# dfm/emcee

Hardware: AMD Instinct MI355X
Metric: walker-updates/sec (whole node), 64-dim correlated Gaussian, StretchMove a=2 (higher is better)
Workload: dtype f64

## Files before the change

### emcee_amd/csrc/emx_kernels.hpp

```cpp
#pragma once
#include <hip/hip_runtime.h>

#include <cstdint>
#include <type_traits>

#include "emx_planlog.hpp"
#include "emx_rng.hpp"

#ifndef EMX_OPT_RED4
#define EMX_OPT_RED4 1
#endif
#ifndef EMX_OPT_RTILE
#define EMX_OPT_RTILE 1
#endif
#ifndef EMX_LEAN_FOLD_D
#define EMX_LEAN_FOLD_D 0
#endif
#ifndef EMX_LEAN_FOLD_SPW
#define EMX_LEAN_FOLD_SPW 1
#endif
#ifndef EMX_OPT_SKEW
#define EMX_OPT_SKEW 1
#endif
#ifndef EMX_SNOOKER_BUDGET
// ... 684 lines not shown
                dst_[e_] = reinterpret_cast<const double2*>(A.tp1)[e_];      \
            __syncthreads();                                                                        \
            stage_pending = false;                                                                  \
        }                                                                                           \
    } while (0)
    const int t_hi = thidev_ ? *thidev_ : A.t_hi;
    if (tlo_ + wave * spw >= t_hi) {
        EMX_STAGE_PUBLISH();
        return;
    }
    for (int t0 = tlo_ + wave * spw; t0 < t_hi; t0 += nwaves * spw) {
        const int nslot = min(spw, t_hi - t0);
        const int npass = (nslot + WPW - 1) / WPW;
        const int pbase = A.pos0 + t0;

        for (int pb = 0; pb < npass; pb += PF) {
            if (skew && stager && stage_pending) {
                EMX_STAGE_PUBLISH();
                for (int r_ = 0; r_ < skewsl_; ++r_) __builtin_amdgcn_s_sleep(8);
            }
            int wi[PF], ja[PF], jb[NR >= 3 ? PF : 1], jc[NR >= 4 ? PF : 1];
#pragma unroll
            for (int k = 0; k < PF; ++k) {
                const int srow = (pb + k) * WPW + sub;
                const int pos = pbase + (srow < nslot ? srow : 0);
                wi[k] = A.order[pos];
                if constexpr (NR >= 2) ja[k] = A.p0[pos];
                if constexpr (NR >= 3) jb[k] = A.p1[pos];
                if constexpr (NR >= 4) jc[k] = A.p2[pos];
            }
            EMX_STAMP(1);
            if (EMX_OPT_STAMPS && A.dbg) {
                asm volatile("s_waitcnt vmcnt(0)" ::: "memory");
                EMX_STAMP(13);
            }
            Row<G, V, CH> xi[PF], xa[NR >= 2 ? PF : 1], xb[NR >= 3 ? PF : 1], xc[NR >= 4 ? PF : 1];
            Row<G, V, CH> qk[RTILE ? PF : 1];
            double s0v[PF], facv[PF], lpov[PF], loguv[PF];
#pragma unroll
            for (int k = 0; k < PF; ++k) {
                const int srow = (pb + k) * WPW + sub;
                const int pos = pbase + (srow < nslot ? srow : 0);
                if (!(ablate_ & 32)) load_row<G, V, CH>(xi[k], A.X + (size_t)wi[k] * D, D, gl);
                if constexpr (MOVE == MOVE_GAUSS) {
                    if (disp_) load_row<G, V, CH>(xa[k], disp_ + (size_t)wi[k] * D, D, gl);
                } else if constexpr (NR >= 2) {
                    if (!(ablate_ & 32)) load_row<G, V, CH>(xa[k], partner_base<LEAN>(A, ja[k]) + (size_t)ja[k] * D, D, gl);
                }
                if constexpr (NR >= 3) load_row<G, V, CH>(xb[k], partner_base<LEAN>(A, jb[k]) + (size_t)jb[k] * D, D, gl);
                if constexpr (NR >= 4) load_row<G, V, CH>(xc[k], partner_base<LEAN>(A, jc[k]) + (size_t)jc[k] * D, D, gl);
                if constexpr (MOVE != MOVE_EVAL) {
                    s0v[k] = (MOVE == MOVE_SNOOKER) ? 0.0 : A.s0[pos];
                    facv[k] = A.fac[pos];
                    if (!DENSE || target_ == TGT_NONE) {
                        lpov[k] = A.lp[wi[k]];
                        loguv[k] = A.logu[pos];
                    } else {
                        lpov[k] = 0.0;
                        loguv[k] = 0.0;
                    }
                } else {
                    s0v[k] = facv[k] = lpov[k] = loguv[k] = 0.0;
                }
            }

            EMX_STAMP(2);
            if (stage_pending) EMX_STAGE_PUBLISH();
            EMX_STAMP(3);

            if (ablate_ & 128) {
                double sink = 0.0;
#pragma unroll
                for (int k = 0; k < PF; ++k) sink += xi[k].x[0][0] + xa[NR >= 2 ? k : 0].x[0][0] + lpov[k];
                if (sink == 1.2345e-300) A.fout[0] = sink;
                continue;
            }
#pragma unroll
            for (int k = 0; k < PF; ++k) {
                const int p = pb + k;
                if (p < npass) {
                    const int srow = p * WPW + sub;
                    const bool live = srow < nslot;
                    const int i = wi[k];
                    double factor = facv[k];

                    Row<G, V, CH> q;
                    if constexpr (MOVE == MOVE_GAUSS)
                        if (!disp_) gauss_disp_row<G, V, CH>(xa[k], A, i, ja[k], D, gl);
                    make_proposal<G, V, CH, MOVE>(xi[k], xa[NR >= 2 ? k : 0], xb[NR >= 3 ? k : 0], xc[NR >= 4 ? k : 0],
                                                  s0v[k], A.gammas, D, gl, q, factor, NR >= 2 ? ja[k] : -1);

                    bool badq = false;
                    if constexpr (MOVE != MOVE_EVAL) {
                        bool bl = false;
#pragma unroll
                        for (int c = 0; c < CH; ++c)
#pragma unroll
                            for (int v = 0; v < V; ++v) bl |= !(fabs(q.x[c][v]) <= 1.79769313486231570815e308);
                        badq = group_any<G>(bl, sub);
                        if (live && badq && gl == 0) raise_status(A.status, ST_BAD_COORD);
                    }

                    if (target_ == TGT_NONE) {
                        if (live) {
                            const int t = t0 + srow;
                            store_row<G, V, CH>(q, A.qout + (size_t)t * D, D, gl);
                            if (gl == 0) A.fout[t] = factor;
                        }
                    } else if (LEAN != 1 && !DENSE && target_ == TGT_REPLAY) {
                        if constexpr (MOVE != MOVE_EVAL) {
                            if (live) {
                                store_row<G, V, CH>(q, A.X + (size_t)i * D, D, gl);
                                if (gl == 0) A.lp[i] = loguv[k];
                            }
                        }
                    } else if constexpr (!DENSE) {
                        const double lp_new = eval_valu_target<G, V, CH>(q, mu, iv, A.tp0, A.tp1, target_, A.tscale, D, gl, lane);
                        if (live && gl == 0 && (lp_new != lp_new)) raise_status(A.status, ST_NAN_LOGP);
                        if constexpr (MOVE == MOVE_EVAL) {
                            if (live && gl == 0) A.lp[i] = lp_new;
                        } else {
                            const double lp_old = lpov[k];
                            const double lnpdiff = factor + lp_new - lp_old;
                            const bool accept = live && !badq && (lnpdiff > loguv[k]);
                            if (accept) {
                                store_row<G, V, CH>(q, A.X + (size_t)i * D, D, gl);
                                if (gl == 0) A.lp[i] = lp_new;
                            }
                            if (live && gl == 0) {
                                A.acc[i] = accept ? 1 : 0;
                                if (chain_lp_) {
                                    chain_lp_[i] = accept ? lp_new : lp_old;
                                    if (accept) A.acc_count[i] += 1u;
                                }
                                if (declp_) put_decision(t0 + srow - tlo_, accept ? lp_new : __builtin_nan(""));
                            }
                            if (live && chain_) store_row_stream<G, V, CH>(accept ? q : xi[k], chain_ + (size_t)i * D, D, gl);
                            if (live && sendbuf_) {
                                double* sb = sendbuf_ + (size_t)(t0 + srow - tlo_) * (D + 2);
                                store_row<G, V, CH>(accept ? q : xi[k], sb, D, gl);
                                if (gl == 0) {
                                    sb[D] = accept ? lp_new : lp_old;
                                    sb[D + 1] = accept ? 1.0 : 0.0;
                                }
                            }
                        }
                    } else {
                        const int trow = srow & 15;
#pragma unroll
                        for (int c = 0; c < CH; ++c)
#pragma unroll
                            for (int v = 0; v < V; ++v) {
                                const int d = (c * G + gl) * V + v;
                                if constexpr (RTILE) {
                                    if (d < Dp && !(ablate_ & 4)) tile[trow * RT + d] = (live && !badq) ? q.x[c][v] - mu.x[c][v] : 0.0;
                                } else {
                                    if (d < Dp && !(ablate_ & 4)) tile[trow * RT + d] = (live && !badq) ? q.x[c][v] : muS[d];
                                }
                            }
                        if constexpr (RTILE) qk[k] = q;
                        if (gl == 0) facS[trow] = badq ? -__builtin_inf() : factor;
                        if constexpr (MOVE != MOVE_EVAL) {
                            if (live && chain_) store_row_stream<G, V, CH>(xi[k], chain_ + (size_t)i * D, D, gl);
                            if (live && sendbuf_)
                                store_row<G, V, CH>(xi[k], sendbuf_ + (size_t)(t0 + srow - tlo_) * (D + 2), D, gl);
                        }
                    }
                }
            }

            EMX_STAMP(4);
            if constexpr (DENSE) {
                const int plast = (pb + PF < npass ? pb + PF : npass) - 1;
                const bool tile_done = ((plast + 1) % PPT == 0) || (plast + 1 == npass);
                if (target_ != TGT_NONE && tile_done && !(ablate_ & 16)) {
                    const int tb = (plast / PPT) * 16;
                    const int myrow = (lane >> 4) + 4 * (lane & 3);
                    const bool mine = (lane & 15) < 4 && tb + myrow < nslot;
                    const int mypos = pbase + (tb + myrow < nslot ? tb + myrow : 0);
                    const int my_i = A.order[mypos];
                    double my_lpo = 0.0, my_logu = 0.0;
                    if constexpr (MOVE != MOVE_EVAL) {
                        my_lpo = A.lp[my_i];
                        my_logu = A.logu[mypos];
                    }
                    EMX_WAVE_SYNC();
                    double my_qf = 0.0;
                    {
                        const int am = lane & 15, ak = lane >> 4;
                        typedef double d4 __attribute__((ext_vector_type(4)));
                        double afr[KK];
#pragma unroll
                        for (int kk = 0; kk < KK; ++kk) {
                            if constexpr (RTILE)
                                afr[kk] = tile[am * RT + 4 * kk + ak];
                            else
                                afr[kk] = tile[am * RT + 4 * kk + ak] - muS[4 * kk + ak];
                        }
                        double part[4] = {0.0, 0.0, 0.0, 0.0};
                        if (EMX_OPT_STAMPS && A.dbg) { asm volatile("s_waitcnt lgkmcnt(0)" ::: "memory"); }
                        EMX_STAMP(5);
                        if (!(ablate_ & 1))
#pragma unroll
                        for (int nb = 0; nb < DPB; ++nb) {
                            d4 accv = {0.0, 0.0, 0.0, 0.0};
#pragma unroll
                            for (int kk = 4 * nb; kk < KK; ++kk)
                                accv = __builtin_amdgcn_mfma_f64_16x16x4f64(afr[kk], Sfrag[(dense_block(DPB, nb, kk >> 2) * 4 + (kk & 3)) * 64 + lane], accv, 0, 0, 0);
#pragma unroll
                            for (int r = 0; r < 4; ++r) part[r] = fma(accv[r], accv[r], part[r]);
                        }
                        if (EMX_OPT_STAMPS && A.dbg) { asm volatile("s_nop 0" ::: "memory"); }
                        EMX_STAMP(6);
#if EMX_OPT_RED4
                        my_qf = row16_sum4(part[0], part[1], part[2], part[3], lane);
#else
#pragma unroll
                        for (int r = 0; r < 4; ++r) part[r] = group_sum<16>(part[r]);
                        my_qf = part[0];
#pragma unroll
                        for (int r = 1; r < 4; ++r) my_qf = (am == r) ? part[r] : my_qf;
#endif
                    }
                    EMX_STAMP(7);
                    bool acc = false;
                    double lp_fin = my_lpo;
                    if (mine) {
                        const double lpn = -0.5 * my_qf;
                        if (lpn != lpn) raise_status(A.status, ST_NAN_LOGP);
                        if constexpr (MOVE == MOVE_EVAL) {
                            A.lp[my_i] = lpn;
                        } else {
                            const double lnpdiff = facS[myrow] + lpn - my_lpo;
                            acc = lnpdiff > my_logu;
                            A.acc[my_i] = acc ? 1 : 0;
                            if (acc) {
                                A.lp[my_i] = lpn;
                                lp_fin = lpn;
                            }
                            if (chain_lp_) {
                                chain_lp_[my_i] = lp_fin;
                                if (acc) A.acc_count[my_i] += 1u;
                            }
                            if (declp_) put_decision(t0 + tb + myrow - tlo_, acc ? lpn : __builtin_nan(""));
                        }
                    }
                    EMX_STAMP(8);
                    if constexpr (MOVE != MOVE_EVAL) {
                        const unsigned long long am64 = __ballot(acc);
                        if (sendbuf_ && (lane & 15) < 4) qfS[myrow] = lp_fin;
                        if (sendbuf_) EMX_WAVE_SYNC();
#pragma unroll
                        for (int pp = 0; pp < PPT; ++pp) {
                            if (ablate_ & 8) break;
                            const int row = pp * WPW + sub;
                            const int sidx = tb + row;
                            const bool lv = sidx < nslot;
                            const bool ac = lv && ((am64 >> ((row & 3) * 16 + (row >> 2))) & 1ull);
                            if (!lv) continue;
                            if (sendbuf_ && gl == 0) {
                                double* sb = sendbuf_ + (size_t)(t0 + sidx - tlo_) * (D + 2);
                                sb[D] = qfS[row];
                                sb[D + 1] = ac ? 1.0 : 0.0;
                            }
                            if (!ac) continue;
                            int wi2;
                            if constexpr (PF == PPT) {
                                wi2 = wi[0];
#pragma unroll
                                for (int k2 = 1; k2 < PF; ++k2) wi2 = (pp == k2) ? wi[k2] : wi2;
                            } else {
                                wi2 = A.order[pbase + sidx];
                            }
                            Row<G, V, CH> rr;
                            if constexpr (RTILE) {
                                rr = qk[pp < PF ? pp : 0];
                            } else {
#pragma unroll
                                for (int c = 0; c < CH; ++c)
#pragma unroll
                                    for (int v = 0; v < V; ++v) {
                                        const int d = (c * G + gl) * V + v;
                                        rr.x[c][v] = d < D ? tile[row * RT + d] : 0.0;
                                    }
                            }
                            store_row<G, V, CH>(rr, A.X + (size_t)wi2 * D, D, gl);
                            if (chain_) store_row_stream<G, V, CH>(rr, chain_ + (size_t)wi2 * D, D, gl);
                            if (sendbuf_) store_row<G, V, CH>(rr, sendbuf_ + (size_t)(t0 + sidx - tlo_) * (D + 2), D, gl);
                        }
                    }
                    EMX_STAMP(9);
                    EMX_WAVE_SYNC();
                }
            }
        }
    }
    if (EMX_OPT_STAMPS && A.dbg) { asm volatile("s_waitcnt vmcnt(0)" ::: "memory"); }
    EMX_STAMP(10);
    if (EMX_OPT_STAMPS && A.dbg && wib == 0 && lane == 0) A.dbg[(size_t)blockIdx.x * 16 + 12] = wall_clock64();
}

typedef unsigned int emx_u4 __attribute__((ext_vector_type(4)));
constexpr int EMX_CPOL_SC1 = 16;
template <int G, int V, int CH, int CPOL = EMX_CPOL_SC1>
__device__ __forceinline__ void load_row_agent(Row<G, V, CH>& r, __amdgpu_buffer_rsrc_t rsrc, int row, int D, int gl) {
    static_assert(V == 2 || V == 1, "two coordinates per lane and chunk (even ndim), or one (odd ndim: rows are 8-byte aligned only)");
    const int base = row * D;
    if constexpr (V == 1) {
        typedef unsigned int emx_u2 __attribute__((ext_vector_type(2)));
#pragma unroll
        for (int c = 0; c < CH; ++c) {
            const int d = c * G + gl;
            if (d < D) {
                const emx_u2 w = __builtin_amdgcn_raw_buffer_load_b64(rsrc, (base + d) * 8, 0, CPOL);
                double t;
                __builtin_memcpy(&t, &w, 8);
                r.x[c][0] = t;
            } else {
                r.x[c][0] = 0.0;
            }
        }
        return;
    }
#pragma unroll
    for (int c = 0; c < CH; ++c) {
        const int d = (c * G + gl) * V;
        if (d + 1 < D) {
            const emx_u4 w = __builtin_amdgcn_raw_buffer_load_b128(rsrc, (base + d) * 8, 0, CPOL);
            double2 t;
            __builtin_memcpy(&t, &w, 16);
            r.x[c][0] = t.x;
            r.x[c][1] = t.y;
        } else {
            r.x[c][0] = 0.0;
            r.x[c][1] = 0.0;
        }
    }
}
template <int G, int V, int CH, int CPOL = EMX_CPOL_SC1>
__device__ __forceinline__ void store_row_agent(const Row<G, V, CH>& r, __amdgpu_buffer_rsrc_t rsrc, int row, int D, int gl) {
    static_assert(V == 2 || V == 1, "two coordinates per lane and chunk (even ndim), or one (odd ndim)");
    const int base = row * D;
    if constexpr (V == 1) {
        typedef unsigned int emx_u2 __attribute__((ext_vector_type(2)));
#pragma unroll
        for (int c = 0; c < CH; ++c) {
            const int d = c * G + gl;
            if (d < D) {
                emx_u2 w;
                const double t = r.x[c][0];
                __builtin_memcpy(&w, &t, 8);
                __builtin_amdgcn_raw_buffer_store_b64(w, rsrc, (base + d) * 8, 0, CPOL);
            }
        }
        return;
    }
#pragma unroll
    for (int c = 0; c < CH; ++c) {
        const int d = (c * G + gl) * V;
        if (d + 1 < D) {
            const double2 t = {r.x[c][0], r.x[c][1]};
            emx_u4 w;
            __builtin_memcpy(&w, &t, 16);
            __builtin_amdgcn_raw_buffer_store_b128(w, rsrc, (base + d) * 8, 0, CPOL);
        }
    }
}
template <typename T>
__device__ __forceinline__ void store_agent(T* p, T v) { __hip_atomic_store(p, v, __ATOMIC_RELAXED, __HIP_MEMORY_SCOPE_AGENT); }
__device__ __forceinline__ double load_agent(const double* p) { return __hip_atomic_load(p, __ATOMIC_RELAXED, __HIP_MEMORY_SCOPE_AGENT); }
__device__ __forceinline__ unsigned load_agent(const unsigned* p) { return __hip_atomic_load(p, __ATOMIC_RELAXED, __HIP_MEMORY_SCOPE_AGENT); }
template <bool LOCAL, typename T>
__device__ __forceinline__ void store_scope(T* p, T v) {
    if constexpr (LOCAL)
        *p = v;
    else
        store_agent(p, v);
}

constexpr int PERSIST_MAX_ITERS = 40;
constexpr int PERSIST_BAR_STRIDE = 32;
constexpr int PERSIST_BAR_WORDS = 12 * PERSIST_BAR_STRIDE;
struct PersistIter {
    const char* plan;
    double *chain, *chain_lp;
    int32_t pos0, split;
    double gammas;
    int32_t kind, shift;
};
struct PersistCols {
    const int32_t *order, *p0, *p1, *p2;
    const double *s0, *logu, *fac;
    double *chain, *chain_lp;
    int32_t pos0, split;
    double gammas;
    int32_t kind, shift;
    __host__ __device__ __forceinline__ PersistCols(const PersistIter& it, size_t N)
        : order(reinterpret_cast<const int32_t*>(it.plan)), p0(reinterpret_cast<const int32_t*>(it.plan) + N),
          p1(reinterpret_cast<const int32_t*>(it.plan + N * 24)), p2(reinterpret_cast<const int32_t*>(it.plan + N * 24) + N),
          s0(reinterpret_cast<const double*>(it.plan + N * 8)), logu(reinterpret_cast<const double*>(it.plan + N * 32)),
          fac(reinterpret_cast<const double*>(it.plan + N * 32) + N), chain(it.chain), chain_lp(it.chain_lp), pos0(it.pos0), split(it.split),
          gammas(it.gammas), kind(it.kind), shift(it.shift) {}
};
struct PersistArgs {
    HalfStepArgs base;
    PersistIter it[PERSIST_MAX_ITERS];
    unsigned* bar;
    unsigned* ver;
    unsigned epoch0;
    unsigned lepoch0;
    unsigned hepoch0;
    unsigned long long timeout_ticks;
    int32_t niter;
    unsigned seq;
    unsigned* started_host;
    int32_t stagger;
};
static_assert(sizeof(PersistArgs) <= 4096, "kernel arguments of the persistent kernels");

__device__ __forceinline__ void persist_barrier_local(const PersistArgs& P, unsigned k, unsigned bid, unsigned ngroups) {
    asm volatile("s_waitcnt vmcnt(0)" ::: "memory");
    __syncthreads();
    if (threadIdx.x < 64) {
        const int lane = threadIdx.x;
        const __amdgpu_buffer_rsrc_t Fr = __builtin_amdgcn_make_buffer_rsrc((void*)(P.bar + 10 * PERSIST_BAR_STRIDE), 0, 64 * 4, 0x00020000);
        if (lane == 0) __builtin_amdgcn_raw_buffer_store_b32(k, Fr, (int)bid * 4, 0, 0);
        const unsigned long long t0 = wall_clock64();
        for (;;) {
            const unsigned v = __builtin_amdgcn_raw_buffer_load_b32(Fr, lane * 4, 0, EMX_CPOL_SC1);
            const bool ok = lane < (int)ngroups ? (int)(v - k) >= 0 : true;
            const bool dead = lane == 32 && v != 0u;
            if (__ballot(ok) == ~0ull || __ballot(dead) != 0ull) break;
            if (wall_clock64() - t0 > P.timeout_ticks) {
                if (lane == 0) {
                    raise_status(P.base.status, ST_EXCHANGE_TIMEOUT);
                    __hip_atomic_store(P.bar + 9 * PERSIST_BAR_STRIDE + 1, 2u, __ATOMIC_RELAXED, __HIP_MEMORY_SCOPE_AGENT);
                    __builtin_amdgcn_raw_buffer_store_b32(1u, Fr, 32 * 4, 0, 0);
                }
                break;
            }
        }
    }
    __syncthreads();
}

__device__ __forceinline__ void persist_barrier(const PersistArgs& P, unsigned k, unsigned long long* wall = nullptr) {
    asm volatile("s_waitcnt vmcnt(0)" ::: "memory");
    __syncthreads();
    if (threadIdx.x == 0) {
        const int xcd = blockIdx.x & 7;
        const unsigned per = (gridDim.x + 7 - xcd) / 8;
        unsigned* xctr = P.bar + xcd * PERSIST_BAR_STRIDE;
        unsigned* gctr = P.bar + 8 * PERSIST_BAR_STRIDE;
        unsigned* go = P.bar + 9 * PERSIST_BAR_STRIDE;
        if (wall) wall[0] = wall_clock64();
        const unsigned old = __hip_atomic_fetch_add(xctr, 1u, __ATOMIC_RELAXED, __HIP_MEMORY_SCOPE_AGENT);
        if (old == k * per - 1) {
            const unsigned o2 = __hip_atomic_fetch_add(gctr, 1u, __ATOMIC_RELAXED, __HIP_MEMORY_SCOPE_AGENT);
            if (o2 == k * 8 - 1) __hip_atomic_store(go, k, __ATOMIC_RELAXED, __HIP_MEMORY_SCOPE_AGENT);
        }
        const unsigned long long t0 = wall_clock64();
        for (;;) {
            const unsigned long long v = __hip_atomic_load(reinterpret_cast<unsigned long long*>(go), __ATOMIC_RELAXED, __HIP_MEMORY_SCOPE_AGENT);
            if ((int)((unsigned)v - k) >= 0 || (v >> 32) != 0ull) break;
            if (wall_clock64() - t0 > P.timeout_ticks) {
                raise_status(P.base.status, ST_EXCHANGE_TIMEOUT);
                __hip_atomic_store(go + 1, 2u, __ATOMIC_RELAXED, __HIP_MEMORY_SCOPE_AGENT);
                break;
            }
        }
        if (wall) wall[1] = wall_clock64();
    }
    __syncthreads();
}

__device__ __forceinline__ void persist_stagger_wait(int stagger, int wib) {
    const int how = stagger >> 8, cnt = stagger & 255;
    const int units = how == 0 ? (wib >> 2) : how == 1 ? (wib & 1) : how == 2 ? ((wib >> 1) & 1) : (wib & 3);
    for (int s = 0; s < cnt * units; ++s) __builtin_amdgcn_s_sleep(1);
}

template <bool LOCAL = false>
__device__ __forceinline__ bool persist_handshake(const PersistArgs& P) {
    __shared__ int ok_s;
    if (threadIdx.x == 0) {
        const unsigned k = LOCAL ? P.hepoch0 + 1u : P.epoch0 + 1u;
        const int xcd = LOCAL ? 0 : (int)(blockIdx.x & 7);
        const unsigned per = LOCAL ? gridDim.x >> 3 : (gridDim.x + 7 - xcd) / 8;
        unsigned* xctr = P.bar + xcd * PERSIST_BAR_STRIDE;
        unsigned* gctr = P.bar + 8 * PERSIST_BAR_STRIDE;
        unsigned* go = P.bar + 9 * PERSIST_BAR_STRIDE;
        int ok = 1;
        const unsigned long long v0 = __hip_atomic_load(reinterpret_cast<unsigned long long*>(go), __ATOMIC_RELAXED, __HIP_MEMORY_SCOPE_AGENT);
        if ((v0 >> 32) != 0ull) {
            ok = 0;
        } else {
            unsigned xcc = 0;
            if constexpr (LOCAL) {
                asm volatile("s_getreg_b32 %0, hwreg(HW_REG_XCC_ID)" : "=s"(xcc));
                __hip_atomic_fetch_or(go + 2, 1u << (xcc & 15u), __ATOMIC_RELAXED, __HIP_MEMORY_SCOPE_AGENT);
                asm volatile("s_waitcnt vmcnt(0)" ::: "memory");
            }
            const unsigned old = __hip_atomic_fetch_add(xctr, 1u, __ATOMIC_RELAXED, __HIP_MEMORY_SCOPE_AGENT);
            if (old == k * per - 1) {
                bool open = true;
                unsigned o2 = k * 8 - 1;
                if constexpr (LOCAL) {
                    const unsigned m = __hip_atomic_load(go + 2, __ATOMIC_RELAXED, __HIP_MEMORY_SCOPE_AGENT);
                    open = (m & (m - 1u)) == 0u;
                    if (open) {
                        __hip_atomic_store(go + 2, 0u, __ATOMIC_RELAXED, __HIP_MEMORY_SCOPE_AGENT);
                    } else {
                        raise_status(P.base.status, ST_EXCHANGE_TIMEOUT);
                        __hip_atomic_store(go + 1, 1u, __ATOMIC_RELAXED, __HIP_MEMORY_SCOPE_AGENT);
                    }
                } else {
                    o2 = __hip_atomic_fetch_add(gctr, 1u, __ATOMIC_RELAXED, __HIP_MEMORY_SCOPE_AGENT);
                }
                if (open && o2 == k * 8 - 1) {
                    __hip_atomic_store(go + 4, LOCAL ? (xcc & 15u) + 1u : 0u, __ATOMIC_RELAXED, __HIP_MEMORY_SCOPE_AGENT);
                    __hip_atomic_store(go + 3, P.seq, __ATOMIC_RELAXED, __HIP_MEMORY_SCOPE_AGENT);
                    if (P.started_host) __hip_atomic_store(P.started_host, P.seq, __ATOMIC_RELAXED, __HIP_MEMORY_SCOPE_SYSTEM);
                    __hip_atomic_store(go, k, __ATOMIC_RELAXED, __HIP_MEMORY_SCOPE_AGENT);
                }
            }
            const unsigned long long t0 = wall_clock64();
            for (;;) {
                const unsigned long long v = __hip_atomic_load(reinterpret_cast<unsigned long long*>(go), __ATOMIC_RELAXED, __HIP_MEMORY_SCOPE_AGENT);
                if ((v >> 32) != 0ull) {
                    ok = 0;
                    break;
                }
                if ((int)((unsigned)v - k) >= 0) break;
                if (wall_clock64() - t0 > P.timeout_ticks) {
                    raise_status(P.base.status, ST_EXCHANGE_TIMEOUT);
                    __hip_atomic_store(go + 1, 1u, __ATOMIC_RELAXED, __HIP_MEMORY_SCOPE_AGENT);
                    ok = 0;
                    break;
                }
            }
        }
        ok_s = ok;
    }
    __syncthreads();
    return ok_s != 0;
}

template <int G, int V, int CH, int DPB, int MOVE = MOVE_STRETCH, bool LOCAL = false, bool ROWS_LATE = false>
static __global__ __launch_bounds__(512) void k_persist(const PersistArgs P) {
    static_assert(MOVE == MOVE_STRETCH || MOVE == MOVE_DE || MOVE == MOVE_SNOOKER, "the red / blue moves");
    if (LOCAL && (blockIdx.x & 7u) != 0u) return;
    const unsigned bid = LOCAL ? blockIdx.x >> 3 : blockIdx.x, ngroups = LOCAL ? gridDim.x >> 3 : gridDim.x;
    constexpr int CPOL = EMX_CPOL_SC1;
    constexpr int CPOL_ST = LOCAL ? 0 : EMX_CPOL_SC1;
    constexpr bool DE = MOVE == MOVE_DE || MOVE == MOVE_SNOOKER;
    constexpr bool SN = MOVE == MOVE_SNOOKER;
    constexpr bool DEFER = !DE;
    constexpr int WPW = 64 / G;
    constexpr int PPT = 16 / WPW;
    constexpr int PF = PPT;
    static_assert(EMX_OPT_RTILE && EMX_OPT_RED4, "the persistent kernel is the one-tile-per-batch form");
    constexpr int Dp = DPB * 16, KK = Dp / 4, RT = Dp + 2;
    static_assert(G * V * CH >= Dp, "row layout must cover the padded dimension");
    extern __shared__ __attribute__((aligned(16))) double smem[];
    const HalfStepArgs& A = P.base;
    const int lane = threadIdx.x & 63;
    const int wib = threadIdx.x >> 6;
    const int sub = lane / G;
    const int gl = lane % G;
    const int D = A.D;
    double* Sfrag = smem;
    double* muS = smem + dense_img_doubles(Dp);
    double* tile = muS + Dp + (size_t)wib * (16 * RT + 32);
    double* qfS = tile + 16 * RT;
    double* facS = qfS + 16;
    {
        constexpr int IMG2 = (dense_img_doubles(Dp) + Dp) / 2;
        const double2* img = reinterpret_cast<const double2*>(A.tp1);
        double2* dst = reinterpret_cast<double2*>(smem);
        for (int e = threadIdx.x; e < IMG2; e += blockDim.x) dst[e] = img[e];
    }
    Row<G, V, CH> mu;
    load_row<G, V, CH>(mu, A.tp0, D, gl);
    if (!persist_handshake<LOCAL>(P)) return;
    const int wave = (int)bid * (blockDim.x >> 6) + wib;
    const int t0 = wave * 16;
    unsigned long long pst[6] = {0, 0, 0, 0, 0, 0}, pt = 0;
    const bool prof = EMX_OPT_STAMPS && A.dbg && wib == EMX_STAMP_WAVE;
    if (prof) {
        pt = __builtin_readcyclecounter();
        if (lane == 0) A.dbg[(size_t)bid * 16 + 11] = wall_clock64();
    }
#define EMX_PSTAMP(k_)                                                   \
    do {                                                                 \
        if (prof) {                                                      \
            const unsigned long long t_ = __builtin_readcyclecounter(); \
            pst[k_] += t_ - pt;                                          \
            pt = t_;                                                     \
        }                                                                \
    } while (0)
    const __amdgpu_buffer_rsrc_t Xr = __builtin_amdgcn_make_buffer_rsrc((void*)A.X, 0, A.N * D * 8, 0x00020000);
    const int myrow = (lane >> 4) + 4 * (lane & 3);
    const bool mine = (lane & 15) < 4;

    int wi[PF], ja[PF], jb[DE ? PF : 1], jc[SN ? PF : 1], my_i;
    double s0v[PF], facv[PF], my_logu, my_lpo;
    Row<G, V, CH> xi[PF];
    {
        const PersistCols I(P.it[0], (size_t)P.base.N);
        const int pbase = I.pos0 + t0;
#pragma unroll
        for (int k = 0; k < PF; ++k) {
            const int pos = pbase + k * WPW + sub;
            wi[k] = I.order[pos];
            ja[k] = I.p0[pos];
            if constexpr (DE) jb[k] = I.p1[pos];
            if constexpr (SN) jc[k] = I.p2[pos];
            s0v[k] = SN ? 0.0 : I.s0[pos];
            facv[k] = I.fac[pos];
        }
        my_i = I.order[pbase + myrow];
        my_logu = I.logu[pbase + myrow];
#pragma unroll
        for (int k = 0; k < PF; ++k) load_row_agent<G, V, CH, CPOL>(xi[k], Xr, wi[k], D, gl);
        my_lpo = load_agent(A.lp + my_i);
    }
    Row<G, V, CH> crow[DEFER ? PF : 1];
    int cwi[PF], cmy_i = 0;
    double clp = 0.0;
    double *cchain = nullptr, *cchain_lp = nullptr;
#pragma unroll
    for (int k = 0; k < PF; ++k) {
        if (DEFER || k == 0) crow[DEFER ? k : 0] = xi[k];
        cwi[k] = 0;
    }
    for (int n = 0; n < P.niter; ++n) {
        const PersistCols I(P.it[n], (size_t)P.base.N);
        Row<G, V, CH> xa[PF], xb[DE ? PF : 1], xc[SN ? PF : 1];
        persist_stagger_wait(P.stagger, wib);
#pragma unroll
        for (int k = 0; k < PF; ++k) {
            load_row_agent<G, V, CH, CPOL>(xa[k], Xr, ja[k], D, gl);
            if constexpr (DE) load_row_agent<G, V, CH, CPOL>(xb[k], Xr, jb[k], D, gl);
            if constexpr (SN) load_row_agent<G, V, CH, CPOL>(xc[k], Xr, jc[k], D, gl);
        }
        const bool more = n + 1 < P.niter;
        const PersistCols J(P.it[more ? n + 1 : n], (size_t)P.base.N);
        const bool pre = more && J.split != 0;
        const unsigned stamp = P.epoch0 + (unsigned)n + 1u;
        int wi_n[PF], ja_n[PF], jb_n[DE ? PF : 1], jc_n[SN ? PF : 1], my_i_n;
        double s0_n[PF], fac_n[PF], my_logu_n;
        {
            const int pbase = J.pos0 + t0;
#pragma unroll
            for (int k = 0; k < PF; ++k) {
                const int pos = pbase + k * WPW + sub;
                wi_n[k] = J.order[pos];
                ja_n[k] = J.p0[pos];
                if constexpr (DE) jb_n[k] = J.p1[pos];
                if constexpr (SN) jc_n[k] = J.p2[pos];
                s0_n[k] = SN ? 0.0 : J.s0[pos];
                fac_n[k] = J.fac[pos];
            }
            my_i_n = J.order[pbase + myrow];
            my_logu_n = J.logu[pbase + myrow];
        }
        if (prof) { asm volatile("s_waitcnt vmcnt(0)" ::: "memory"); }
        EMX_PSTAMP(0);
        Row<G, V, CH> qk[PF];
#pragma unroll
        for (int k = 0; k < PF; ++k) {
            const int srow = k * WPW + sub;
            double factor = facv[k];
            Row<G, V, CH> q;
            make_proposal<G, V, CH, MOVE>(xi[k], xa[k], xb[DE ? k : 0], xc[SN ? k : 0], s0v[k], A.gammas, D, gl, q, factor, ja[k]);
            bool bl = false;
#pragma unroll
            for (int c = 0; c < CH; ++c)
#pragma unroll
                for (int v = 0; v < V; ++v) bl |= !(fabs(q.x[c][v]) <= 1.79769313486231570815e308);
            const bool badq = group_any<G>(bl, sub);
            if (badq && gl == 0) raise_status(A.status, ST_BAD_COORD);
            const int trow = srow & 15;
#pragma unroll
            for (int c = 0; c < CH; ++c)
#pragma unroll
                for (int v = 0; v < V; ++v) {
                    const int d = (c * G + gl) * V + v;
                    if (d < Dp) tile[trow * RT + d] = !badq ? q.x[c][v] - mu.x[c][v] : 0.0;
                }
            qk[k] = q;
            if (gl == 0) facS[trow] = badq ? -__builtin_inf() : factor;
        }
        if (DEFER && cchain) {
#pragma unroll
            for (int k = 0; k < PF; ++k) store_row_stream<G, V, CH>(crow[k], cchain + (size_t)cwi[k] * D, D, gl);
            if (mine) cchain_lp[cmy_i] = clp;
            cchain = nullptr;
        }
        if (I.chain) {
#pragma unroll
            for (int k = 0; k < PF; ++k) {
                if constexpr (DEFER)
                    crow[k] = xi[k];
                else
                    store_row_stream<G, V, CH>(xi[k], I.chain + (size_t)wi[k] * D, D, gl);
            }
        }
        double my_lpo_n = 0.0;
        if (!ROWS_LATE && more) {
#pragma unroll
            for (int k = 0; k < PF; ++k) load_row_agent<G, V, CH, CPOL>(xi[k], Xr, wi_n[k], D, gl);
            my_lpo_n = load_agent(A.lp + my_i_n);
        }
        EMX_WAVE_SYNC();
        EMX_PSTAMP(1);
        double my_qf;
        {
            const int am = lane & 15, ak = lane >> 4;
            typedef double d4 __attribute__((ext_vector_type(4)));
            double afr[KK];
#pragma unroll
            for (int kk = 0; kk < KK; ++kk) afr[kk] = tile[am * RT + 4 * kk + ak];
            double part[4] = {0.0, 0.0, 0.0, 0.0};
#pragma unroll
            for (int nb = 0; nb < DPB; ++nb) {
                d4 accv = {0.0, 0.0, 0.0, 0.0};
#pragma unroll
                for (int kk = 4 * nb; kk < KK; ++kk)
                    accv = __builtin_amdgcn_mfma_f64_16x16x4f64(afr[kk], Sfrag[(dense_block(DPB, nb, kk >> 2) * 4 + (kk & 3)) * 64 + lane], accv, 0, 0, 0);
#pragma unroll
                for (int r = 0; r < 4; ++r) part[r] = fma(accv[r], accv[r], part[r]);
            }
            my_qf = row16_sum4(part[0], part[1], part[2], part[3], lane);
        }
        if (ROWS_LATE && more) {
            __builtin_amdgcn_sched_barrier(0);
#pragma unroll
            for (int k = 0; k < PF; ++k) load_row_agent<G, V, CH, CPOL>(xi[k], Xr, wi_n[k], D, gl);
            my_lpo_n = load_agent(A.lp + my_i_n);
            __builtin_amdgcn_sched_barrier(0);
        }
        if (prof) { asm volatile("s_nop 0" ::: "memory"); }
        EMX_PSTAMP(2);
        bool acc = false;
        if (mine) {
            const double lpn = -0.5 * my_qf;
            if (lpn != lpn) raise_status(A.status, ST_NAN_LOGP);
            const double lnpdiff = facS[myrow] + lpn - my_lpo;
            acc = lnpdiff > my_logu;
            store_scope<LOCAL>(A.acc + my_i, (uint8_t)(acc ? 1 : 0));
            if (acc) {
                store_scope<LOCAL>(A.lp + my_i, lpn);
                store_scope<LOCAL>(P.ver + my_i, stamp);
            }
            if (I.chain_lp) {
                if constexpr (DEFER)
                    clp = acc ? lpn : my_lpo;
                else
                    I.chain_lp[my_i] = acc ? lpn : my_lpo;
                if (acc) store_scope<LOCAL>(A.acc_count + my_i, load_agent(A.acc_count + my_i) + 1u);
            }
        }
        const unsigned long long am64 = __ballot(acc);
#pragma unroll
        for (int pp = 0; pp < PPT; ++pp) {
            const int row = pp * WPW + sub;
            const bool ac = (am64 >> ((row & 3) * 16 + (row >> 2))) & 1ull;
            if (ac) {
                store_row_agent<G, V, CH, CPOL_ST>(qk[pp], Xr, wi[pp], D, gl);
                if (I.chain) {
                    if constexpr (DEFER)
                        crow[pp] = qk[pp];
                    else
                        store_row_stream<G, V, CH>(qk[pp], I.chain + (size_t)wi[pp] * D, D, gl);
                }
            }
        }
        if (DEFER && I.chain) {
            cchain = I.chain;
            cchain_lp = I.chain_lp;
            cmy_i = my_i;
#pragma unroll
            for (int k = 0; k < PF; ++k) cwi[k] = wi[k];
        }
        EMX_WAVE_SYNC();
        EMX_PSTAMP(3);
        if (prof) {
            asm volatile("s_waitcnt vmcnt(0)" ::: "memory");
            EMX_PSTAMP(4);
        }
        if (!more) break;
        if constexpr (LOCAL)
            persist_barrier_local(P, P.lepoch0 + (unsigned)n + 1u, bid, ngroups);
        else
            persist_barrier(P, P.epoch0 + (unsigned)n + 2u,
                            (EMX_OPT_STAMPS && A.dbg) ? A.dbg + 4096 + ((size_t)n * ngroups + bid) * 2 : nullptr);
        EMX_PSTAMP(5);
#pragma unroll
        for (int k = 0; k < PF; ++k) {
            wi[k] = wi_n[k];
            ja[k] = ja_n[k];
            if constexpr (DE) jb[k] = jb_n[k];
            if constexpr (SN) jc[k] = jc_n[k];
            s0v[k] = s0_n[k];
            facv[k] = fac_n[k];
        }
        my_i = my_i_n;
        my_logu = my_logu_n;
        my_lpo = my_lpo_n;
        if (!pre) {
            unsigned vk[PF];
#pragma unroll
            for (int k = 0; k < PF; ++k) vk[k] = load_agent(P.ver + wi[k]);
            const unsigned vm = load_agent(P.ver + my_i);
#pragma unroll
            for (int k = 0; k < PF; ++k)
                if (vk[k] == stamp) load_row_agent<G, V, CH, CPOL>(xi[k], Xr, wi[k], D, gl);
            if (vm == stamp) my_lpo = load_agent(A.lp + my_i);
        }
    }
    if (DEFER && cchain) {
#pragma unroll
        for (int k = 0; k < PF; ++k) store_row_stream<G, V, CH>(crow[k], cchain + (size_t)cwi[k] * D, D, gl);
        if (mine) cchain_lp[cmy_i] = clp;
    }
    if (prof && lane == 0) {
        unsigned long long* o = A.dbg + (size_t)bid * 16;
#pragma unroll
        for (int k = 0; k < 6; ++k) o[k] = pst[k];
        o[6] = (unsigned long long)P.niter;
        o[12] = wall_clock64();
    }
#undef EMX_PSTAMP
}

constexpr int SMALL_MAX_MOVES = 8;
struct GaussGen {
    unsigned long long gseed, gstep;
    double gfac, gsigma;
    const double* gscale;
};
constexpr int PERSIST_GAUSS_MAX_STEPS = 16;
struct PersistGaussStep {
    const int32_t* p0;
    const double* logu;
    double *chain, *chain_lp;
    unsigned long long gstep;
    double gfac;
};
struct PersistGaussArgs {
    HalfStepArgs base;
    PersistGaussStep st[PERSIST_GAUSS_MAX_STEPS];
    int32_t nsteps;
};

template <int G, int V, int CH, int DPB>
static __global__ __launch_bounds__(512) void k_persist_gauss(const PersistGaussArgs P) {
    constexpr int MOVE = MOVE_GAUSS;
    constexpr int WPW = 64 / G;
    constexpr int PPT = 16 / WPW;
    constexpr int Dp = DPB * 16, KK = Dp / 4, RT = Dp + 2;
    static_assert(EMX_OPT_RTILE && EMX_OPT_RED4 && G * V * CH >= Dp, "the one-tile-per-batch form");
    extern __shared__ __attribute__((aligned(16))) double smem[];
    const HalfStepArgs& A = P.base;
    const int lane = threadIdx.x & 63;
    const int wib = threadIdx.x >> 6;
    const int sub = lane / G;
    const int gl = lane % G;
    const int D = A.D;
    double* Sfrag = smem;
    double* muS = smem + dense_img_doubles(Dp);
    double* tile = muS + Dp + (size_t)wib * (16 * RT + 32);
    double* facS = tile + 16 * RT + 16;
    {
        constexpr int IMG2 = (dense_img_doubles(Dp) + Dp) / 2;
        const double2* img = reinterpret_cast<const double2*>(A.tp1);
        double2* dst = reinterpret_cast<double2*>(smem);
        for (int e = threadIdx.x; e < IMG2; e += blockDim.x) dst[e] = img[e];
    }
    Row<G, V, CH> mu;
    load_row<G, V, CH>(mu, A.tp0, D, gl);
    __syncthreads();
    const int wave = blockIdx.x * (blockDim.x >> 6) + wib;
    const int w0 = wave * 16;
    const int myrow = (lane >> 4) + 4 * (lane & 3);
    const bool mine = (lane & 15) < 4;
    const int my_i = w0 + myrow;
    Row<G, V, CH> xi[PPT];
#pragma unroll
    for (int k = 0; k < PPT; ++k) load_row<G, V, CH>(xi[k], A.X + (size_t)(w0 + k * WPW + sub) * D, D, gl);
    double my_lp = A.lp[my_i];
    bool my_acc = false;
    for (int s = 0; s < P.nsteps; ++s) {
        const PersistGaussStep& S = P.st[s];
        GaussGen gg;
        gg.gseed = A.gseed;
        gg.gstep = S.gstep;
        gg.gfac = S.gfac;
        gg.gsigma = A.gsigma;
        gg.gscale = A.gscale;
        const double my_logu = S.logu[my_i];
        Row<G, V, CH> qk[PPT];
#pragma unroll
        for (int k = 0; k < PPT; ++k) {
            const int i = w0 + k * WPW + sub;
            const int col = S.p0[i];
            Row<G, V, CH> xa, q;
            gauss_disp_row<G, V, CH>(xa, gg, i, col, D, gl);
            double factor = 0.0;
            make_proposal<G, V, CH, MOVE>(xi[k], xa, xa, xa, 0.0, A.gammas, D, gl, q, factor, col);
            bool bl = false;
#pragma unroll
            for (int c = 0; c < CH; ++c)
#pragma unroll
                for (int v = 0; v < V; ++v) bl |= !(fabs(q.x[c][v]) <= 1.79769313486231570815e308);
            const bool badq = group_any<G>(bl, sub);
            if (badq && gl == 0) raise_status(A.status, ST_BAD_COORD);
            const int trow = (k * WPW + sub) & 15;
#pragma unroll
            for (int c = 0; c < CH; ++c)
#pragma unroll
                for (int v = 0; v < V; ++v) {
                    const int d = (c * G + gl) * V + v;
                    if (d < Dp) tile[trow * RT + d] = !badq ? q.x[c][v] - mu.x[c][v] : 0.0;
                }
            qk[k] = q;
            if (gl == 0) facS[trow] = badq ? -__builtin_inf() : factor;
        }
        EMX_WAVE_SYNC();
        double my_qf;
        {
            const int am = lane & 15, ak = lane >> 4;
            typedef double d4 __attribute__((ext_vector_type(4)));
            double afr[KK];
#pragma unroll
            for (int kk = 0; kk < KK; ++kk) afr[kk] = tile[am * RT + 4 * kk + ak];
            double part[4] = {0.0, 0.0, 0.0, 0.0};
#pragma unroll
            for (int nb = 0; nb < DPB; ++nb) {
                d4 accv = {0.0, 0.0, 0.0, 0.0};
#pragma unroll
                for (int kk = 4 * nb; kk < KK; ++kk)
                    accv = __builtin_amdgcn_mfma_f64_16x16x4f64(afr[kk], Sfrag[(dense_block(DPB, nb, kk >> 2) * 4 + (kk & 3)) * 64 + lane], accv, 0, 0, 0);
#pragma unroll
                for (int r = 0; r < 4; ++r) part[r] = fma(accv[r], accv[r], part[r]);
            }
            my_qf = row16_sum4(part[0], part[1], part[2], part[3], lane);
        }
        bool acc = false;
        if (mine) {
            const double lpn = -0.5 * my_qf;
            if (lpn != lpn) raise_status(A.status, ST_NAN_LOGP);
            const double lnpdiff = facS[myrow] + lpn - my_lp;
            acc = lnpdiff > my_logu;
            if (acc) my_lp = lpn;
            my_acc = acc;
            if (S.chain_lp) {
                S.chain_lp[my_i] = my_lp;
                if (acc) A.acc_count[my_i] += 1u;
            }
        }
        const unsigned long long am64 = __ballot(acc);
#pragma unroll
        for (int pp = 0; pp < PPT; ++pp) {
            const int row = pp * WPW + sub;
            const bool ac = (am64 >> ((row & 3) * 16 + (row >> 2))) & 1ull;
            if (ac) xi[pp] = qk[pp];
            if (S.chain) store_row_stream<G, V, CH>(xi[pp], S.chain + (size_t)(w0 + row) * D, D, gl);
        }
        EMX_WAVE_SYNC();
    }
#pragma unroll
    for (int k = 0; k < PPT; ++k) store_row<G, V, CH>(xi[k], A.X + (size_t)(w0 + k * WPW + sub) * D, D, gl);
    if (mine) {
        A.lp[my_i] = my_lp;
        A.acc[my_i] = my_acc ? 1 : 0;
    }
}

constexpr int SMALL_ANY_MOVE = 7;

__host__ __device__ inline int native_move_choice(uint64_t seed, uint64_t step, const double* cdf, int n) {
    const Philox4 r = philox4x32_10((uint32_t)step, (uint32_t)(step >> 32), 0x4d4f5645u , 0, (uint32_t)seed,
                                    (uint32_t)(seed >> 32));
    const double u = u53(r.v[0], r.v[1]);
    int k = 0;
    while (k < n - 1 && u >= cdf[k]) ++k;
    return k;
}

struct SmallRunArgs {
    double* X;
    double* lp;
    uint8_t* acc;
    uint32_t* acc_count;
    uint32_t* status;
    double* chain;
    double* chain_lp;
    const double* tp0;
    const double* tp1;
    double tscale;
    double a[SMALL_MAX_MOVES], sigma[SMALL_MAX_MOVES], g0[SMALL_MAX_MOVES], gammas[SMALL_MAX_MOVES], cdf[SMALL_MAX_MOVES];
    int32_t kind[SMALL_MAX_MOVES], nsplits[SMALL_MAX_MOVES];
    int32_t gmode[SMALL_MAX_MOVES];
    double gsigma[SMALL_MAX_MOVES];
    const double* gscale[SMALL_MAX_MOVES];
    const double* step_fac;
    const int32_t* step_col;
    int32_t nmoves;
    unsigned long long seed, step0;
    long long i0;
    int32_t N, D, target, nsteps, thin_by, store;
    int32_t batch;
    const char* plans;
    const int32_t* step_moves;
    const unsigned long long* seeds;
    const double* tscales;
    long long tp0_stride, tp1_stride, cap;
    int32_t eval0;
    const void* user;
    int32_t stage_rows;
};

constexpr int SMALL_STATUS_WORDS = 8;

template <bool BATCH>
struct SmallMember {
    const SmallRunArgs& A;
    __device__ __forceinline__ size_t m() const { return BATCH ? (size_t)blockIdx.x : 0; }
    __device__ __forceinline__ double* X() const { return A.X + m() * (size_t)A.N * A.D; }
    __device__ __forceinline__ double* lp() const { return A.lp + m() * (size_t)A.N; }
    __device__ __forceinline__ uint8_t* acc() const { return A.acc + m() * (size_t)A.N; }
    __device__ __forceinline__ uint32_t* acc_count() const { return A.acc_count + m() * (size_t)A.N; }
    __device__ __forceinline__ uint32_t* status() const { return A.status + m() * SMALL_STATUS_WORDS; }
    __device__ __forceinline__ double* chain() const { return A.chain + m() * (size_t)A.cap * A.N * A.D; }
    __device__ __forceinline__ double* chain_lp() const { return A.chain_lp + m() * (size_t)A.cap * A.N; }
    __device__ __forceinline__ const double* tp0() const { return BATCH && A.tp0 ? A.tp0 + m() * (size_t)A.tp0_stride : A.tp0; }
    __device__ __forceinline__ const double* tp1() const { return BATCH && A.tp1 ? A.tp1 + m() * (size_t)A.tp1_stride : A.tp1; }
    __device__ __forceinline__ const double* step_fac() const { return BATCH && A.step_fac ? A.step_fac + m() * (size_t)A.nsteps : A.step_fac; }
    __device__ __forceinline__ double tscale() const { return BATCH ? A.tscales[m()] : A.tscale; }
    __device__ __forceinline__ unsigned long long seed() const { return BATCH ? A.seeds[m()] : A.seed; }
};

template <int MOVE>
__device__ __forceinline__ void small_plan_entry(const NativeArgs& na, int N, int D, int S, int pos, double a, double sigma,
                                                 double g0, int& i, int& a0, int& a1, int& a2, double& z, double& lu, double& fc) {
    int split = 0, t = pos;
    const SplitSizes sz = split_sizes(N, S);
    for (int k = 0; k < S; ++k) {
        const int n = sz.of(k);
        if (t < n) { split = k; break; }
        t -= n;
    }
    double u;
    native_slot<MOVE>(na, N, S, split, t, a, sigma, g0, i, a0, a1, a2, z, u);
    lu = plan_log_uniform(u);
    fc = (MOVE == MOVE_STRETCH) ? ((double)D - 1.0) * plan_log(z) : 0.0;
}

template <int G, int V, int CH, int MOVE, typename Member>
__device__ __forceinline__ void small_propose(const Member& M, const double* Xs, bool live, int i, int j0, int j1, int j2,
                                              double s0, double fac, double gammas, int D, int gl, int sub, Row<G, V, CH>& q,
                                              double& factor, bool& badq, const GaussGen* gg = nullptr) {
    constexpr int NR = rows_per_pass<MOVE>();
    Row<G, V, CH> xi, xa, xb, xc;
    load_row<G, V, CH>(xi, Xs + (size_t)i * D, D, gl);
    if constexpr (MOVE == MOVE_GAUSS)
        gauss_disp_row<G, V, CH>(xa, *gg, i, j0, D, gl);
    else
        load_row<G, V, CH>(xa, Xs + (size_t)j0 * D, D, gl);
    if constexpr (NR >= 3) load_row<G, V, CH>(xb, Xs + (size_t)j1 * D, D, gl);
    if constexpr (NR >= 4) load_row<G, V, CH>(xc, Xs + (size_t)j2 * D, D, gl);
    factor = fac;
    make_proposal<G, V, CH, MOVE>(xi, xa, NR >= 3 ? xb : xa, NR >= 4 ? xc : xa, (MOVE == MOVE_SNOOKER) ? 0.0 : s0, gammas, D,
                                  gl, q, factor, MOVE == MOVE_GAUSS ? j0 : -1);
    bool bl = false;
#pragma unroll
    for (int c = 0; c < CH; ++c)
#pragma unroll
        for (int v = 0; v < V; ++v) bl |= !(fabs(q.x[c][v]) <= 1.79769313486231570815e308);
    badq = group_any<G>(bl, sub);
    if (live && badq && gl == 0) raise_status(M.status(), ST_BAD_COORD);
}

template <int G, int V, int CH, int MOVE, typename Member>
__device__ __forceinline__ void small_update(const SmallRunArgs& A, const Member& M, double* Xs, double* lps, uint8_t* accs, bool live, int i,
                                             int j0, int j1, int j2, double s0, double fac, double logu, double gammas,
                                             const Row<G, V, CH>& mu, const Row<G, V, CH>& iv, int D, int gl, int sub, int lane,
                                             const GaussGen* gg = nullptr) {
    Row<G, V, CH> q;
    double factor;
    bool badq;
    small_propose<G, V, CH, MOVE>(M, Xs, live, i, j0, j1, j2, s0, fac, gammas, D, gl, sub, q, factor, badq, gg);
    const double lp_new = eval_valu_target<G, V, CH>(q, mu, iv, M.tp0(), M.tp1(), A.target, M.tscale(), D, gl, lane);
    if (live && gl == 0 && (lp_new != lp_new)) raise_status(M.status(), ST_NAN_LOGP);
    const double lp_old = lps[i];
    const double lnpdiff = factor + lp_new - lp_old;
    const bool accept = live && !badq && (lnpdiff > logu);
    if (accept) {
        store_row<G, V, CH>(q, Xs + (size_t)i * D, D, gl);
        if (gl == 0) lps[i] = lp_new;
    }
    if (live && gl == 0) accs[i] = accept ? 1 : 0;
}

template <typename USER>
__device__ __forceinline__ double fused_call(const double* x, int ndim, int member, const void* user) {
    if constexpr (std::is_void<USER>::value) {
        return 0.0;
    } else {
        return USER{}(x, ndim, member, user);
    }
}

template <int DPB, int KK, int RT>
__device__ __forceinline__ double small_dense_qf(const double* tile, const double* muS, const double* Sfrag, int lane) {
    double qf;
    const int am = lane & 15, ak = lane >> 4;
    typedef double d4 __attribute__((ext_vector_type(4)));
    double afr[KK];
#pragma unroll
    for (int kk = 0; kk < KK; ++kk) afr[kk] = tile[am * RT + 4 * kk + ak] - muS[4 * kk + ak];
    double part[4] = {0.0, 0.0, 0.0, 0.0};
#pragma unroll
    for (int nb = 0; nb < DPB; ++nb) {
        d4 accv = {0.0, 0.0, 0.0, 0.0};
#pragma unroll
        for (int kk = 4 * nb; kk < KK; ++kk)
            accv = __builtin_amdgcn_mfma_f64_16x16x4f64(afr[kk], Sfrag[(dense_block(DPB, nb, kk >> 2) * 4 + (kk & 3)) * 64 + lane], accv, 0, 0, 0);
#pragma unroll
        for (int r = 0; r < 4; ++r) part[r] = fma(accv[r], accv[r], part[r]);
    }
#if EMX_OPT_RED4
    qf = row16_sum4(part[0], part[1], part[2], part[3], lane);
#else
#pragma unroll
// ... 1136 lines not shown
```

Before: 3.346 billion.

## Defer post-barrier version check into next iteration, overlapped with partner row loads

Moves the version-stamp check and conditional reload of the walker's own row and log-prob from after the grid barrier to the start of the next iteration. The version loads are issued first and the partner-row loads are issued before waiting on them, so the latency of the check overlaps the complementary-ensemble fetch. Adds a COUNTED variant of the row loader that always issues the buffer load and masks with a select, avoiding branches so the loads can be counted and kept in flight. Profiling stamps are also extended to split boundary and non-boundary iterations.

Result: slower. 3.300 billion (-1.4%).

```diff
diff --git a/emcee_amd/csrc/emx_kernels.hpp b/emcee_amd/csrc/emx_kernels.hpp
--- a/emcee_amd/csrc/emx_kernels.hpp
+++ b/emcee_amd/csrc/emx_kernels.hpp
@@ -1010,10 +1010,35 @@
 
 typedef unsigned int emx_u4 __attribute__((ext_vector_type(4)));
 constexpr int EMX_CPOL_SC1 = 16;
-template <int G, int V, int CH, int CPOL = EMX_CPOL_SC1>
+template <int G, int V, int CH, int CPOL = EMX_CPOL_SC1, bool COUNTED = false>
 __device__ __forceinline__ void load_row_agent(Row<G, V, CH>& r, __amdgpu_buffer_rsrc_t rsrc, int row, int D, int gl) {
     static_assert(V == 2 || V == 1, "two coordinates per lane and chunk (even ndim), or one (odd ndim: rows are 8-byte aligned only)");
     const int base = row * D;
+    if constexpr (COUNTED && V == 1) {
+        typedef unsigned int emx_u2 __attribute__((ext_vector_type(2)));
+#pragma unroll
+        for (int c = 0; c < CH; ++c) {
+            const int d = c * G + gl;
+            const emx_u2 w = __builtin_amdgcn_raw_buffer_load_b64(rsrc, (base + d) * 8, 0, CPOL);
+            double t;
+            __builtin_memcpy(&t, &w, 8);
+            r.x[c][0] = d < D ? t : 0.0;
+        }
+        return;
+    }
+    if constexpr (COUNTED && V == 2) {
+#pragma unroll
+        for (int c = 0; c < CH; ++c) {
+            const int d = (c * G + gl) * V;
+            const bool in = d + 1 < D;
+            const emx_u4 w = __builtin_amdgcn_raw_buffer_load_b128(rsrc, (base + d) * 8, 0, CPOL);
+            double2 t;
+            __builtin_memcpy(&t, &w, 16);
+            r.x[c][0] = in ? t.x : 0.0;
+            r.x[c][1] = in ? t.y : 0.0;
+        }
+        return;
+    }
     if constexpr (V == 1) {
         typedef unsigned int emx_u2 __attribute__((ext_vector_type(2)));
 #pragma unroll
@@ -1293,7 +1318,8 @@
     if (!persist_handshake<LOCAL>(P)) return;
     const int wave = (int)bid * (blockDim.x >> 6) + wib;
     const int t0 = wave * 16;
-    unsigned long long pst[6] = {0, 0, 0, 0, 0, 0}, pt = 0;
+    unsigned long long pst[6] = {0, 0, 0, 0, 0, 0}, pstb[6] = {0, 0, 0, 0, 0, 0}, pchk = 0, pt = 0;
+    bool pbnd = true;
     const bool prof = EMX_OPT_STAMPS && A.dbg && wib == EMX_STAMP_WAVE;
     if (prof) {
         pt = __builtin_readcyclecounter();
@@ -1303,7 +1329,16 @@
     do {                                                                 \
         if (prof) {                                                      \
             const unsigned long long t_ = __builtin_readcyclecounter(); \
-            pst[k_] += t_ - pt;                                          \
+            pst[k_] += pbnd ? 0ull : t_ - pt;                            \
+            pstb[k_] += pbnd ? t_ - pt : 0ull;                           \
+            pt = t_;                                                     \
+        }                                                                \
+    } while (0)
+#define EMX_PSTAMP_CHECK()                                               \
+    do {                                                                 \
+        if (prof) {                                                      \
+            const unsigned long long t_ = __builtin_readcyclecounter(); \
+            pchk += t_ - pt;                                             \
             pt = t_;                                                     \
         }                                                                \
     } while (0)
@@ -1342,15 +1377,31 @@
         if (DEFER || k == 0) crow[DEFER ? k : 0] = xi[k];
         cwi[k] = 0;
     }
+    bool chk = false;
+    unsigned pstamp = 0u;
     for (int n = 0; n < P.niter; ++n) {
         const PersistCols I(P.it[n], (size_t)P.base.N);
+        if (EMX_OPT_STAMPS) pbnd = I.split == 0;
+        unsigned vk[PF] = {}, vm = 0u;
+        if (chk) {
+#pragma unroll
+            for (int k = 0; k < PF; ++k) vk[k] = load_agent(P.ver + wi[k]);
+            vm = load_agent(P.ver + my_i);
+        }
         Row<G, V, CH> xa[PF], xb[DE ? PF : 1], xc[SN ? PF : 1];
         persist_stagger_wait(P.stagger, wib);
 #pragma unroll
         for (int k = 0; k < PF; ++k) {
-            load_row_agent<G, V, CH, CPOL>(xa[k], Xr, ja[k], D, gl);
-            if constexpr (DE) load_row_agent<G, V, CH, CPOL>(xb[k], Xr, jb[k], D, gl);
-            if constexpr (SN) load_row_agent<G, V, CH, CPOL>(xc[k], Xr, jc[k], D, gl);
+            load_row_agent<G, V, CH, CPOL, true>(xa[k], Xr, ja[k], D, gl);
+            if constexpr (DE) load_row_agent<G, V, CH, CPOL, true>(xb[k], Xr, jb[k], D, gl);
+            if constexpr (SN) load_row_agent<G, V, CH, CPOL, true>(xc[k], Xr, jc[k], D, gl);
+        }
+        if (chk) {
+            if (vm == pstamp) my_lpo = load_agent(A.lp + my_i);
+#pragma unroll
+            for (int k = 0; k < PF; ++k)
+                if (vk[k] == pstamp) load_row_agent<G, V, CH, CPOL>(xi[k], Xr, wi[k], D, gl);
+            EMX_PSTAMP_CHECK();
         }
         const bool more = n + 1 < P.niter;
         const PersistCols J(P.it[more ? n + 1 : n], (size_t)P.base.N);
@@ -1517,16 +1568,8 @@
         my_i = my_i_n;
         my_logu = my_logu_n;
         my_lpo = my_lpo_n;
-        if (!pre) {
-            unsigned vk[PF];
-#pragma unroll
-            for (int k = 0; k < PF; ++k) vk[k] = load_agent(P.ver + wi[k]);
-            const unsigned vm = load_agent(P.ver + my_i);
-#pragma unroll
-            for (int k = 0; k < PF; ++k)
-                if (vk[k] == stamp) load_row_agent<G, V, CH, CPOL>(xi[k], Xr, wi[k], D, gl);
-            if (vm == stamp) my_lpo = load_agent(A.lp + my_i);
-        }
+        chk = !pre;
+        pstamp = stamp;
     }
     if (DEFER && cchain) {
 #pragma unroll
@@ -1536,11 +1579,16 @@
     if (prof && lane == 0) {
         unsigned long long* o = A.dbg + (size_t)bid * 16;
 #pragma unroll
-        for (int k = 0; k < 6; ++k) o[k] = pst[k];
+        for (int k = 0; k < 6; ++k) {
+            o[k] = pst[k];
+            o[k < 4 ? 7 + k : 9 + k] = pstb[k];
+        }
         o[6] = (unsigned long long)P.niter;
         o[12] = wall_clock64();
+        o[15] = pchk;
     }
 #undef EMX_PSTAMP
+#undef EMX_PSTAMP_CHECK
 }
 
 constexpr int SMALL_MAX_MOVES = 8;
```
